# e4s2024/E4S2024

Hardware: AMD Instinct MI355X
Metric: 1024x1024 faces/sec (StyleGAN2 regional synthesis, gen_img) (higher is better)
Workload: dtype f16+mxfp6x2 (masked 3x3 layers >= 32^2) / bf16x3 (all other layers); 1 GPU; BASELINE configs[1]: StyleGAN2 1024x1024 synthesis from random W+, 12-region masks, batch=4/GPU; batch_per_gpu=4, global_batch=4, parallelism=frames x1, streams_per_gpu=2

## Files before the change

### e4s2024_amd/csrc/modconv_uphc.hip

```cpp
#include <stdlib.h>

#include "common.h"
#include "sb_common.h"

using namespace e4s;

namespace {

struct UpHcParams {
    uint4* out;
    const uint4* x;
    const uint4* whi;
    const uint4* wlo;
    const float* d;
    const float* blur;
    const float* noise;
    const float* noise_weight;
    const float* act_bias;
    const float* s_next;
    const float* zeros;
    int noise_bstride, act;
    int bs, cin, cout, h, w;
    int tiles_x, tiles_y;
    int ntile, ncot;
    int exp;
    int rev;
    int walk;
    int64_t plane_in, plane_out;
};

constexpr int HC_T = 16;
constexpr int HC_STEP = HC_T - 2;
constexpr int HC_PW = HC_T + 1, HC_PH = HC_T + 2;
constexpr int HC_PATCH = HC_PW * HC_PH;
constexpr int HC_NT = 512;
constexpr int HC_XB4 = 4 * HC_PATCH;
constexpr int HC_W4 = 36 * 32;
constexpr int HC_BODY = (2 * HC_XB4 + 2 * HC_W4) * 16;
constexpr int HC_EP_D = 0, HC_EP_B = 64, HC_EP_S = 128, HC_EP_FLOATS = 192;
constexpr int HC_LDS = HC_BODY + HC_EP_FLOATS * 4;
constexpr int HC_G = 3;
static_assert(HC_LDS <= 80 * 1024, "two workgroups per CU");

template <int CTRL>
__device__ __forceinline__ float dpp_row(float v) {
    return __builtin_bit_cast(float, __builtin_amdgcn_update_dpp(0, __builtin_bit_cast(int, v), CTRL, 0xf, 0xf, true));
}
constexpr int DPP_ROW_SHL1 = 0x101;
constexpr int DPP_ROW_SHR1 = 0x111;

__device__ __forceinline__ uint4 dpp_row_shr1(uint4 v) {
    uint4 r;
    r.x = (unsigned)__builtin_amdgcn_update_dpp(0, (int)v.x, DPP_ROW_SHR1, 0xf, 0xf, true);
    r.y = (unsigned)__builtin_amdgcn_update_dpp(0, (int)v.y, DPP_ROW_SHR1, 0xf, 0xf, true);
    r.z = (unsigned)__builtin_amdgcn_update_dpp(0, (int)v.z, DPP_ROW_SHR1, 0xf, 0xf, true);
    r.w = (unsigned)__builtin_amdgcn_update_dpp(0, (int)v.w, DPP_ROW_SHR1, 0xf, 0xf, true);
    return r;
}
template <int PAR>
__device__ __forceinline__ void hc_unit(f32x16 (&accs)[4], const uint4* xs, const uint4* whalf) {
    uint4 bh[2], bl[2], ah[2], al[2];
    auto fetch_b = [&](int dyi, int slot) __attribute__((always_inline)) {
        bh[slot] = xs[dyi * HC_PW + 1];
        bl[slot] = xs[2 * HC_PATCH + dyi * HC_PW + 1];
    };
    auto fetch_a = [&](int tap, int slot) __attribute__((always_inline)) {
        ah[slot] = whalf[tap * 64];
        al[slot] = whalf[18 * 32 + tap * 64];
    };
    fetch_b(0, 0);
    fetch_a(0, 0);
#pragma unroll
    for (int dyi = 0; dyi < 3; ++dyi) {
        const int bs = dyi & 1;
        if (dyi + 1 < 3) fetch_b(dyi + 1, bs ^ 1);
        const uint4 sh = dpp_row_shr1(bh[bs]), sl = dpp_row_shr1(bl[bs]);
#pragma unroll
        for (int kx = 0; kx < 3; ++kx) {
            const int tap = dyi * 3 + kx, cs = tap & 1;
            if (tap + 1 < 9) fetch_a(tap + 1, cs ^ 1);
            const uint4 xh = kx == 2 ? sh : bh[bs], xl = kx == 2 ? sl : bl[bs];
            const int ai = 2 * PAR + (kx & 1);
            accs[ai] = __builtin_amdgcn_mfma_f32_32x32x16_bf16(__builtin_bit_cast(bf16x8, ah[cs]), __builtin_bit_cast(bf16x8, xh), accs[ai], 0, 0, 0);
            accs[ai] = __builtin_amdgcn_mfma_f32_32x32x16_bf16(__builtin_bit_cast(bf16x8, ah[cs]), __builtin_bit_cast(bf16x8, xl), accs[ai], 0, 0, 0);
            accs[ai] = __builtin_amdgcn_mfma_f32_32x32x16_bf16(__builtin_bit_cast(bf16x8, al[cs]), __builtin_bit_cast(bf16x8, xh), accs[ai], 0, 0, 0);
            __builtin_amdgcn_sched_barrier(0);
        }
    }
}

E4S_PROF_DECL(g_prof_hc)

__device__ __forceinline__ void hc_epilogue(const UpHcParams& p, const f32x16 (&accs)[4], const unsigned char* lds_raw, int ep_off, const float2 (&nz)[2], bool lane_ok,
                                            int b, int co0, int pm, int pbx, int khalf) {
    const int ho = 2 * p.h, wo = 2 * p.w;
    float khf[4];
    {
        float cs[4], S = 0.f;
#pragma unroll
        for (int cc = 0; cc < 4; ++cc) { cs[cc] = p.blur[cc] + p.blur[4 + cc] + p.blur[8 + cc] + p.blur[12 + cc]; S += cs[cc]; }
        const float rs = 1.f / sqrtf(S);
#pragma unroll
        for (int u = 0; u < 4; ++u) khf[u] = cs[3 - u] * rs;
    }
    const float nw = p.noise ? p.noise_weight[0] : 0.f;
    const float neg = p.act ? 0.2f : 1.f, gain = p.act ? 1.41421356237309515f : 1.f;
    const size_t opl = (size_t)ho * wo;
    const size_t o_base = ((size_t)b * (p.cout >> 3) + (size_t)(co0 >> 3)) * opl + (size_t)(2 * pm) * wo + (size_t)(2 * pbx + khalf);
#pragma unroll
    for (int g = 0; g < 4; ++g) {
        unsigned ep_i = (unsigned)(ep_off / 4 + 8 * g + 4 * khalf);
        asm volatile("" : "+v"(ep_i));
        const float* ep = reinterpret_cast<const float*>(lds_raw) + ep_i;
        const float4 d4 = *reinterpret_cast<const float4*>(ep + HC_EP_D);
        const float4 b4 = *reinterpret_cast<const float4*>(ep + HC_EP_B);
        const float4 s4 = *reinterpret_cast<const float4*>(ep + HC_EP_S);
        const float dd[4] = {d4.x, d4.y, d4.z, d4.w}, bb[4] = {b4.x, b4.y, b4.z, b4.w}, sn[4] = {s4.x, s4.y, s4.z, s4.w};
#pragma unroll
        for (int pa = 0; pa < 2; ++pa) {
            const float nze = __fmul_rn(nw, nz[pa].x), nzo = __fmul_rn(nw, nz[pa].y);
            float ue[4], uo[4];
#pragma unroll
            for (int j = 0; j < 4; ++j) {
                const float z0 = accs[2 * pa][4 * g + j], z1 = accs[2 * pa + 1][4 * g + j];
                const float l1 = dpp_row<DPP_ROW_SHR1>(z1);
                const float r0 = dpp_row<DPP_ROW_SHL1>(z0);
                const float r1 = dpp_row<DPP_ROW_SHL1>(z1);
                float oe = __fmul_rn(khf[0], l1);
                oe = __builtin_fmaf(khf[1], z0, oe);
                oe = __builtin_fmaf(khf[2], z1, oe);
                oe = __builtin_fmaf(khf[3], r0, oe);
                float oo = __fmul_rn(khf[0], z0);
                oo = __builtin_fmaf(khf[1], z1, oo);
                oo = __builtin_fmaf(khf[2], r0, oo);
                oo = __builtin_fmaf(khf[3], r1, oo);
                float ve = __builtin_fmaf(oe, dd[j], bb[j]) + nze, vo = __builtin_fmaf(oo, dd[j], bb[j]) + nzo;
                ve = fmaxf(ve, ve * neg) * gain;
                vo = fmaxf(vo, vo * neg) * gain;
                ue[j] = __fmul_rn(ve, sn[j]);
                uo[j] = __fmul_rn(vo, sn[j]);
            }
            unsigned he[2], le[2], ho_[2], lo_[2];
            split2(ue[0], ue[1], he[0], le[0]);
            split2(ue[2], ue[3], he[1], le[1]);
            split2(uo[0], uo[1], ho_[0], lo_[0]);
            split2(uo[2], uo[3], ho_[1], lo_[1]);
#pragma unroll
            for (int q = 0; q < 2; ++q) {
                auto r = __builtin_amdgcn_permlane32_swap(he[q], ho_[q], false, false);
                he[q] = r[0]; ho_[q] = r[1];
                auto r2 = __builtin_amdgcn_permlane32_swap(le[q], lo_[q], false, false);
                le[q] = r2[0]; lo_[q] = r2[1];
            }
#ifdef E4S_PHASE_PROF
            if ((p.exp & 4) && he[0] != 0x12345678u) continue;
#endif
            if (lane_ok) {
                const size_t o4 = o_base + (size_t)g * opl + (size_t)pa * wo;
                p.out[o4] = make_uint4(he[0], he[1], ho_[0], ho_[1]);
                p.out[(size_t)p.plane_out + o4] = make_uint4(le[0], le[1], lo_[0], lo_[1]);
            }
        }
    }
}


__global__ __launch_bounds__(HC_NT, 4) void up_hc_kernel(const UpHcParams p) {
    extern __shared__ __attribute__((aligned(16))) unsigned char lds_raw[];
    const uint4* lds4 = reinterpret_cast<const uint4*>(lds_raw);
    const float* epw = reinterpret_cast<const float*>(lds_raw + HC_BODY);
    const int tid = threadIdx.x;
    const int lane = tid & 63;
    const int wave = __builtin_amdgcn_readfirstlane(tid >> 6);
    const int l5 = lane & 31, khalf = lane >> 5;
    E4S_PROF_MARK(g_prof_hc, 0);
    const int tyt = blockIdx.x / p.tiles_x, txt = blockIdx.x - tyt * p.tiles_x;
    const int m0 = tyt * HC_T, p0x = txt * HC_STEP - 1;
    const int co0 = blockIdx.y * 32;
    const int b = blockIdx.z;
    const int hw = p.h * p.w, ho = 2 * p.h, wo = 2 * p.w;
    const int nchunk = p.cin >> 4, cb8 = p.cin >> 3;
    const unsigned zero_off = (unsigned)(2 * p.plane_in * 16);

    const int pty = 2 * wave + (l5 >> 4), ptx = l5 & 15;
    const int pm = m0 + pty, pbx = p0x + ptx;
    const bool lane_ok = ptx >= 1 && ptx <= HC_STEP && pbx < p.w && pm < p.h;
    float2 nz[2] = {make_float2(0.f, 0.f), make_float2(0.f, 0.f)};
    if (p.noise && lane_ok) {
        const float* np = p.noise + (size_t)b * p.noise_bstride + (size_t)(2 * pm) * wo + 2 * pbx;
        nz[0] = *reinterpret_cast<const float2*>(np);
        nz[1] = *reinterpret_cast<const float2*>(np + wo);
    }

    unsigned xoffs[3], xdst[3];
    bool xin[3];
#pragma unroll
    for (int k = 0; k < 3; ++k) {
        int u = wave + 8 * k;
        u = u < 20 ? u : 19;
        const int j = u % 5, combo = u / 5;
        const int e = j * 64 + lane;
        const int py = e / HC_PW, px = e - py * HC_PW;
        const int gy = m0 - 1 + py, gx = p0x - 1 + px;
        xin[k] = e < HC_PATCH && gy >= 0 && gy < p.h && gx >= 0 && gx < p.w;
        xoffs[k] = (unsigned)((combo >> 1) * p.plane_in) + (unsigned)((b * cb8 + (combo & 1)) * hw + gy * p.w + gx);
        xdst[k] = (unsigned)((combo * HC_PATCH + j * 64) * 16);
    }
    auto issue_x = [&](int c) __attribute__((always_inline)) {
        const unsigned st = (unsigned)(c & 1) * (unsigned)(HC_XB4 * 16);
#pragma unroll
        for (int k = 0; k < 3; ++k) {
            const int e = ((wave + 8 * k < 20 ? wave + 8 * k : 19) % 5) * 64 + lane;
            if (e < HC_PATCH) dma16_asm(p.x, xin[k] ? (xoffs[k] + (unsigned)(2 * c * hw)) * 16u : zero_off, st + xdst[k]);
        }
    };
    auto issue_w = [&](int u) __attribute__((always_inline)) {
        const unsigned st = (unsigned)((2 * HC_XB4 + (u & 1) * HC_W4) * 16);
        const int c = u >> 1, par = u & 1;
#pragma unroll
        for (int k = 0; k < 3; ++k) {
            int piece = wave + 8 * k;
            piece = piece < 18 ? piece : 17;
            const int hl = piece / 9;
            const int rem = piece * 64 - hl * 576 + lane;
            dma16_asm(hl ? p.wlo : p.whi, (unsigned)(((((par * nchunk + c) * 18 + (rem >> 5)) * p.cout) + co0 + (rem & 31)) * 16), st + (unsigned)(piece * 1024));
        }
    };
    {
        const unsigned co4 = (unsigned)((co0 + l5) * 4);
        dma4_asm(p.d, (unsigned)(b * p.cout * 4) + co4, (unsigned)(HC_BODY + HC_EP_D * 4));
        dma4_asm(p.s_next, (unsigned)(b * p.cout * 4) + co4, (unsigned)(HC_BODY + HC_EP_S * 4));
        dma4_asm(p.act_bias ? p.act_bias : p.zeros, p.act_bias ? co4 : 0u, (unsigned)(HC_BODY + HC_EP_B * 4));
    }
    issue_x(0);
    issue_w(0);
    issue_w(1);
    if (nchunk > 1) issue_x(1);

    const int xoff = pty * HC_PW + ptx;
    f32x16 accs[4];
#pragma unroll
    for (int a = 0; a < 4; ++a)
#pragma unroll
        for (int r = 0; r < 16; ++r) accs[a][r] = 0.f;

#pragma unroll 1
    for (int c = 0; c < nchunk; ++c) {
        const bool last = c + 1 >= nchunk;
#pragma unroll
        for (int par = 0; par < 2; ++par) {
            if (!last) E4S_WAIT_VM(2 * HC_G);
            else if (par == 0) E4S_WAIT_VM(HC_G);
            else E4S_WAIT_VM(0);
            E4S_LDS_BARRIER();
            if (c == 0 && par == 0) E4S_PROF_MARK(g_prof_hc, 1);
            unsigned xb_i = (unsigned)((c & 1) * HC_XB4 + khalf * HC_PATCH + xoff);
            unsigned wb_i = (unsigned)(2 * HC_XB4 + par * HC_W4 + khalf * 32 + l5);
            asm volatile("" : "+v"(xb_i), "+v"(wb_i));
            const uint4* xs = lds4 + xb_i;
            const uint4* whalf = lds4 + wb_i;
            if (par == 0) hc_unit<0>(accs, xs, whalf); else hc_unit<1>(accs, xs, whalf);
            E4S_LDS_BARRIER();
            if (!last) {
                issue_w(2 * c + par + 2);
                if (par == 1 && c + 2 < nchunk) issue_x(c + 2);
            }
        }
    }
    E4S_PROF_MARK(g_prof_hc, 2);

    E4S_PROF_MARK(g_prof_hc, 3);
    if (blockIdx.x == 0 && blockIdx.y == 0 && blockIdx.z == 0 && tid < 1) p.out[(size_t)p.plane_out * 2] = make_uint4(0u, 0u, 0u, 0u);
    hc_epilogue(p, accs, lds_raw, HC_BODY, nz, lane_ok, b, co0, pm, pbx, khalf);
    E4S_PROF_MARK(g_prof_hc, 4);
    E4S_PROF_DRAIN();
    E4S_PROF_MARK(g_prof_hc, 5);
}


constexpr int HP_NCW = 8;
constexpr int HP_NT = 64 * (HP_NCW + 2);
constexpr int HP_NX = 4, HP_NW = 4;
constexpr int HP_W0 = HP_NX * HC_XB4;
constexpr int HP_BODY = (HP_NX * HC_XB4 + HP_NW * HC_W4) * 16;
constexpr int HP_LDS = HP_BODY + HC_EP_FLOATS * 4;
constexpr int HP_GX = 20, HP_GW = 18;
static_assert(HP_LDS <= 160 * 1024 && (HP_NX - 1) * HP_GX <= 63 && (HP_NW - 1) * HP_GW + 3 <= 63, "LDS per CU; vmcnt is a 6-bit counter");

__global__ __launch_bounds__(HP_NT) void up_hcp_kernel(const UpHcParams p) {
    extern __shared__ __attribute__((aligned(16))) unsigned char lds_raw[];
    const uint4* lds4 = reinterpret_cast<const uint4*>(lds_raw);
    const int tid = threadIdx.x;
    const int lane = tid & 63;
    const int wave = __builtin_amdgcn_readfirstlane(tid >> 6);
    const int hw = p.h * p.w, wo = 2 * p.w;
    const int nchunk = p.cin >> 4, NU = 2 * nchunk;
    const int stride = gridDim.x, first = walk_offset(blockIdx.x, stride, p.walk & 1);
    const int my_tiles = (p.ntile - first + stride - 1) / stride;
    const int my_items = my_tiles * p.ncot;
    const int per_img = p.tiles_x * p.tiles_y;
    const int total = my_items * NU;
    auto item_coords = [&](int i, int& b, int& cot, int& tyt, int& txt) __attribute__((always_inline)) {
        i = i < my_items ? i : my_items - 1;
        int t = first + (i / p.ncot) * stride;
        t = p.rev ? p.ntile - 1 - t : t;
        cot = i % p.ncot;
        b = t / per_img;
        walk_tile_xy(t - b * per_img, p.tiles_x, p.tiles_y, p.walk >> 8, tyt, txt);
    };

    if (wave == HP_NCW) {
        lds_byte* const lds_b = (lds_byte*)lds_raw;
        auto issue_w = [&](int k) __attribute__((always_inline)) {
            const int u = k % NU, c = u >> 1, par = u & 1;
            int b, cot, tyt, txt;
            item_coords(k / NU, b, cot, tyt, txt);
            const unsigned wst = (unsigned)((HP_W0 + (k % HP_NW) * HC_W4) * 16);
#pragma unroll
            for (int piece = 0; piece < HP_GW; ++piece) {
                const int hl = piece / 9;
                const int rem = piece * 64 - hl * 576 + lane;
                dma16(hl ? p.wlo : p.whi, (unsigned)(((((par * nchunk + c) * 18 + (rem >> 5)) * p.cout) + cot * 32 + (rem & 31)) * 16), lds_b + wst + piece * 1024);
            }
        };
        auto item_setup = [&](int i) __attribute__((always_inline)) {
            int b, cot, tyt, txt;
            item_coords(i, b, cot, tyt, txt);
            const unsigned co4 = (unsigned)((cot * 32 + (lane & 31)) * 4);
            dma4(p.d, (unsigned)(b * p.cout * 4) + co4, lds_b + HP_BODY + HC_EP_D * 4);
            dma4(p.s_next, (unsigned)(b * p.cout * 4) + co4, lds_b + HP_BODY + HC_EP_S * 4);
            dma4(p.act_bias ? p.act_bias : p.zeros, p.act_bias ? co4 : 0u, lds_b + HP_BODY + HC_EP_B * 4);
        };
        item_setup(0);
#pragma unroll
        for (int k = 0; k < HP_NW - 1; ++k) issue_w(k);
#pragma unroll 1
        for (int k = 0; k < total; ++k) {
            E4S_WAIT_VM(2 * HP_GW);
            E4S_LDS_BARRIER();
            if (k > 0 && k % NU == 0) item_setup(k / NU);
            issue_w(k + HP_NW - 1);
        }
        E4S_WAIT_VM(0);
        return;
    }
    if (wave == HP_NCW + 1) {
        const int cb8 = p.cin >> 3;
        lds_byte* const lds_b = (lds_byte*)lds_raw;
        const unsigned zero_off = (unsigned)(2 * p.plane_in * 16);
        auto issue_x = [&](int q) __attribute__((always_inline)) {
            const int c = q % nchunk;
            int b, cot, tyt, txt;
            item_coords(q / nchunk, b, cot, tyt, txt);
            const unsigned xst = (unsigned)((q % HP_NX) * (HC_XB4 * 16));
            const int m0 = tyt * HC_T, p0x = txt * HC_STEP - 1;
            const unsigned cb0 = (unsigned)((b * cb8 + 2 * c) * hw);
#pragma unroll
            for (int j = 0; j < 5; ++j) {
                const int e = j * 64 + lane;
                const int py = e / HC_PW, px = e - py * HC_PW;
                const int gy = m0 - 1 + py, gx = p0x - 1 + px;
                const bool inb = gy >= 0 && gy < p.h && gx >= 0 && gx < p.w;
                const unsigned pix = (unsigned)(gy * p.w + gx);
                if (e < HC_PATCH) {
#pragma unroll
                    for (int combo = 0; combo < 4; ++combo) {
                        const unsigned cbase = (unsigned)((combo >> 1) * p.plane_in) + cb0 + (unsigned)((combo & 1) * hw);
                        dma16(p.x, inb ? (cbase + pix) * 16u : zero_off, lds_b + xst + (combo * HC_PATCH + j * 64) * 16);
                    }
                }
            }
        };
#pragma unroll
        for (int q = 0; q < HP_NX - 1; ++q) issue_x(q);
#pragma unroll 1
        for (int k = 0; k < total; ++k) {
            if (k & 1) { E4S_LDS_BARRIER(); continue; }
            E4S_WAIT_VM(2 * HP_GX);
            E4S_LDS_BARRIER();
            issue_x((k >> 1) + HP_NX - 1);
        }
        E4S_WAIT_VM(0);
        return;
    }

    const int l5 = lane & 31, khalf = lane >> 5;
    const int pty = 2 * wave + (l5 >> 4), ptx = l5 & 15;
    const int xoff = pty * HC_PW + ptx;
    if (blockIdx.x == 0 && tid < 1) p.out[(size_t)p.plane_out * 2] = make_uint4(0u, 0u, 0u, 0u);
    int xbuf = 0;
#pragma unroll 1
    for (int ti = 0; ti < my_items; ++ti) {
        int b, cot, tyt, txt;
        item_coords(ti, b, cot, tyt, txt);
        const int pm = tyt * HC_T + pty, pbx = txt * HC_STEP - 1 + ptx;
        const bool lane_ok = ptx >= 1 && ptx <= HC_STEP && pbx < p.w && pm < p.h;
        float2 nz[2] = {make_float2(0.f, 0.f), make_float2(0.f, 0.f)};
        if (p.noise && lane_ok) {
            const float* np = p.noise + (size_t)b * p.noise_bstride + (size_t)(2 * pm) * wo + 2 * pbx;
            nz[0] = *reinterpret_cast<const float2*>(np);
            nz[1] = *reinterpret_cast<const float2*>(np + wo);
        }
        f32x16 accs[4];
#pragma unroll
        for (int a = 0; a < 4; ++a)
#pragma unroll
            for (int r = 0; r < 16; ++r) accs[a][r] = 0.f;
#pragma unroll 1
        for (int c = 0; c < nchunk; ++c) {
#pragma unroll
            for (int par = 0; par < 2; ++par) {
                const int k = ti * NU + 2 * c + par;
                E4S_LDS_BARRIER();
                unsigned xb_i = (unsigned)(xbuf * HC_XB4 + khalf * HC_PATCH + xoff);
                unsigned wb_i = (unsigned)(HP_W0 + (k % HP_NW) * HC_W4 + khalf * 32 + l5);
                asm volatile("" : "+v"(xb_i), "+v"(wb_i));
                const uint4* xs = lds4 + xb_i;
                const uint4* whalf = lds4 + wb_i;
#ifdef E4S_PHASE_PROF
                if (p.exp & 2) continue;
#endif
                if (par == 0) hc_unit<0>(accs, xs, whalf); else hc_unit<1>(accs, xs, whalf);
            }
            xbuf = xbuf + 1 < HP_NX ? xbuf + 1 : 0;
        }
#ifdef E4S_PHASE_PROF
        if (p.exp & 1) { asm volatile("" :: "v"(accs[0][0]), "v"(accs[1][0]), "v"(accs[2][0]), "v"(accs[3][0])); continue; }
#endif
        hc_epilogue(p, accs, lds_raw, HP_BODY, nz, lane_ok, b, cot * 32, pm, pbx, khalf);
    }
}

__global__ __launch_bounds__(256) void prep_weights_hc_kernel(uint16_t* __restrict__ whi, uint16_t* __restrict__ wlo, const float* __restrict__ weight,
                                                              const float* __restrict__ blur, int cout, int cin, float scale) {
    const int nchunk = (cin + CKS - 1) / CKS;
    const int64_t total = (int64_t)2 * nchunk * 9 * 2 * cout * 8;
    float kvf[4];
    {
        float rsum[4], S = 0.f;
#pragma unroll
        for (int r = 0; r < 4; ++r) { rsum[r] = blur[4 * r] + blur[4 * r + 1] + blur[4 * r + 2] + blur[4 * r + 3]; S += rsum[r]; }
        const float rs = 1.f / sqrtf(S);
#pragma unroll
        for (int t = 0; t < 4; ++t) kvf[t] = rsum[3 - t] * rs;
    }
    for (int64_t i = (int64_t)blockIdx.x * 256 + threadIdx.x; i < total; i += (int64_t)gridDim.x * 256) {
        const int e = (int)(i & 7);
        int64_t r = i >> 3;
        const int co = (int)(r % cout); r /= cout;
        const int half = (int)(r & 1); r >>= 1;
        const int tap = (int)(r % 9); r /= 9;
        const int chunk = (int)(r % nchunk);
        const int par = (int)(r / nchunk);
        const int ci = chunk * CKS + half * 8 + e;
        float v = 0.f;
        if (ci < cin) {
            const float* w = weight + ((size_t)co * cin + ci) * 9;
            const int dy = tap / 3 - 1, kx = tap % 3;
#pragma unroll
            for (int ky = 0; ky < 3; ++ky) {
                const int ty = ky + 2 * dy + 1 - par;
                if (ty >= 0 && ty <= 3) v += kvf[ty] * w[ky * 3 + kx];
            }
            v *= scale;
        }
        const unsigned hp = pack_bf16_rne(v, 0.f) & 0xffffu;
        const float hf = __builtin_bit_cast(float, hp << 16);
        whi[i] = (uint16_t)hp;
        wlo[i] = (uint16_t)(pack_bf16_rne(v - hf, 0.f) & 0xffffu);
    }
}

__device__ uint4 g_hc_zero[4];

}

#ifdef E4S_PHASE_PROF
extern "C" E4S_API int e4s_prof_read_hc(long long* host, int64_t n) {
    return (int)hipMemcpyFromSymbol(host, HIP_SYMBOL(g_prof_hc), (size_t)n * sizeof(long long), 0, hipMemcpyDeviceToHost);
}
extern "C" E4S_API int e4s_prof_clear_hc() {
    void* ptr = nullptr;
    hipError_t e = hipGetSymbolAddress(&ptr, HIP_SYMBOL(g_prof_hc));
    if (e != hipSuccess) return (int)e;
    return (int)hipMemset(ptr, 0, sizeof(long long) * (size_t)E4S_PROF_BLOCKS * E4S_PROF_SLOTS);
}
#endif

extern "C" int e4s_modconv_prep_weights_hc(uint16_t* whi, uint16_t* wlo, const float* weight, const float* blur, int cout, int cin, void* stream) {
    E4S_REQUIRE(whi && wlo && weight && blur, "modconv_prep_weights_hc: null tensor");
    E4S_REQUIRE(cout >= 1 && cin >= 1, "modconv_prep_weights_hc: bad channel counts");
    const float scale = 1.0f / sqrtf((float)cin * 9.f);
    const int64_t total = (int64_t)2 * cdiv(cin, CKS) * 9 * 2 * cout * 8;
    const int grid = (int)(cdiv64(total, 256) < 4096 ? cdiv64(total, 256) : 4096);
    hipLaunchKernelGGL(prep_weights_hc_kernel, dim3(grid), dim3(256), 0, (hipStream_t)stream, whi, wlo, weight, blur, cout, cin, scale);
    return check_launch("modconv_prep_weights_hc");
}

extern "C" int e4s_modconv_up_hc(uint16_t* out_sp, const uint16_t* x_sp, const uint16_t* whi, const uint16_t* wlo, const float* d, const float* blur,
                                 const float* noise, int noise_bs, const float* noise_weight, const float* act_bias, int act,
                                 int bs, int cin, int cout, int h, int w, const float* s_next, void* stream) {
    E4S_REQUIRE(out_sp && x_sp && whi && wlo && d && blur && s_next, "modconv_up_hc: null tensor (d and s_next are required)");
    E4S_REQUIRE(bs >= 0 && bs <= 65535 && h >= 1 && w >= 1 && cin >= 16 && cin % 16 == 0 && cout >= 32 && cout % 32 == 0, "modconv_up_hc: bad size (cin %% 16, cout %% 32)");
    E4S_REQUIRE((int64_t)bs * cout * 4 * h * w < ((int64_t)1 << 31) && (int64_t)bs * cin * h * w < ((int64_t)1 << 31), "modconv_up_hc: a tensor must stay below 2^31 elements");
    E4S_REQUIRE((((uintptr_t)out_sp | (uintptr_t)x_sp | (uintptr_t)whi | (uintptr_t)wlo) & 15) == 0, "modconv_up_hc: tensors must be 16-byte aligned");
    E4S_REQUIRE(!noise || (noise_weight && (noise_bs == 1 || noise_bs == bs) && ((uintptr_t)noise & 7) == 0), "modconv_up_hc: noise needs its weight, batch 1 or bs and 8-byte alignment");
    if (bs == 0) return 0;
    static const float* zeros = [] {
        void* ptr = nullptr;
        return hipGetSymbolAddress(&ptr, HIP_SYMBOL(g_hc_zero)) == hipSuccess ? static_cast<const float*>(ptr) : nullptr;
    }();
    static const hipError_t attr = hipFuncSetAttribute(reinterpret_cast<const void*>(&up_hc_kernel), hipFuncAttributeMaxDynamicSharedMemorySize, HC_LDS);
    static const hipError_t attr_p = hipFuncSetAttribute(reinterpret_cast<const void*>(&up_hcp_kernel), hipFuncAttributeMaxDynamicSharedMemorySize, HP_LDS);
    if (!zeros || attr != hipSuccess || attr_p != hipSuccess) return fail(E4S_ERR_ARG, "modconv_up_hc: cannot set up the kernel (zero block / dynamic LDS limit)");
    UpHcParams p;
    p.out = reinterpret_cast<uint4*>(out_sp); p.x = reinterpret_cast<const uint4*>(x_sp);
    p.whi = reinterpret_cast<const uint4*>(whi); p.wlo = reinterpret_cast<const uint4*>(wlo);
    p.d = d; p.blur = blur; p.noise = noise; p.noise_weight = noise_weight; p.act_bias = act_bias; p.s_next = s_next; p.zeros = zeros;
    p.noise_bstride = (noise && noise_bs > 1) ? 4 * h * w : 0;
    p.act = act & 1; p.bs = bs; p.cin = cin; p.cout = cout; p.h = h; p.w = w;
    p.tiles_x = cdiv(2 * w, 2 * HC_STEP); p.tiles_y = cdiv(h, HC_T);
    p.ntile = p.tiles_x * p.tiles_y * bs; p.ncot = cout / 32;
    p.plane_in = (int64_t)bs * (cin / 8) * h * w;
    p.plane_out = (int64_t)bs * (cout / 8) * 4 * h * w;
    static const int rev = [] { const char* e = getenv("E4S_HC_REV"); return e ? atoi(e) : 1; }();
    static const int walk = [] { const char* e = getenv("E4S_WALK"); return e ? atoi(e) : (1 | (8 << 8)); }();
    p.rev = rev; p.walk = walk;
#ifdef E4S_PHASE_PROF
    { const char* e = getenv("E4S_HC_EXP"); p.exp = e ? atoi(e) : 0; }
#else
    p.exp = 0;
#endif
    if (cin >= 32) {
        static const int ncu = [] {
            int dev = 0, n = 256;
            if (hipGetDevice(&dev) == hipSuccess) (void)hipDeviceGetAttribute(&n, hipDeviceAttributeMultiprocessorCount, dev);
            return n > 0 ? n : 256;
        }();
        hipLaunchKernelGGL(up_hcp_kernel, dim3(p.ntile < ncu ? p.ntile : ncu), dim3(HP_NT), HP_LDS, (hipStream_t)stream, p);
        return check_launch("modconv_up_hc");
    }
    hipLaunchKernelGGL(up_hc_kernel, dim3(p.tiles_x * p.tiles_y, cout / 32, bs), dim3(HC_NT), HC_LDS, (hipStream_t)stream, p);
    return check_launch("modconv_up_hc");
}
```

Before: 1509 faces/s.

## Use wide 32x8 tiles with wave-level DPP shifts in persistent upsample modconv

The persistent upsample-conv kernel switches from a 16-wide, two-rows-per-wave tile to a 32-wide tile with one tile row per wave. Horizontal neighbour shifts now use wave-wide DPP instead of row DPP, so halo overhead per tile drops and patch loads become whole 64-lane pieces. Leftover tiles are also split at item (tile x cout-tile) granularity across persistent workgroups to balance the tail. Risks include changed LDS footprint, edge handling of wave-wide shifts across the 32-lane halves, and more complex index math.

```diff
diff --git a/e4s2024_amd/csrc/modconv_uphc.hip b/e4s2024_amd/csrc/modconv_uphc.hip
--- a/e4s2024_amd/csrc/modconv_uphc.hip
+++ b/e4s2024_amd/csrc/modconv_uphc.hip
@@ -48,21 +48,37 @@
 }
 constexpr int DPP_ROW_SHL1 = 0x101;
 constexpr int DPP_ROW_SHR1 = 0x111;
-
-__device__ __forceinline__ uint4 dpp_row_shr1(uint4 v) {
+constexpr int DPP_WAVE_SHL1 = 0x130;
+constexpr int DPP_WAVE_SHR1 = 0x138;
+
+constexpr int HP_TW = 32, HP_TH = 8;
+constexpr int HP_STEP = HP_TW - 2;
+constexpr int HP_PW = HP_TW, HP_PH = HP_TH + 2;
+constexpr int HP_PATCH = HP_PW * HP_PH;
+template <bool WIDE> struct HcGeo;
+template <> struct HcGeo<false> {
+    static constexpr int PW = HC_PW, PATCH = HC_PATCH, XO = 1, SHR1 = DPP_ROW_SHR1, SHL1 = DPP_ROW_SHL1;
+};
+template <> struct HcGeo<true> {
+    static constexpr int PW = HP_PW, PATCH = HP_PATCH, XO = 0, SHR1 = DPP_WAVE_SHR1, SHL1 = DPP_WAVE_SHL1;
+};
+
+template <int CTRL>
+__device__ __forceinline__ uint4 dpp_shr1(uint4 v) {
     uint4 r;
-    r.x = (unsigned)__builtin_amdgcn_update_dpp(0, (int)v.x, DPP_ROW_SHR1, 0xf, 0xf, true);
-    r.y = (unsigned)__builtin_amdgcn_update_dpp(0, (int)v.y, DPP_ROW_SHR1, 0xf, 0xf, true);
-    r.z = (unsigned)__builtin_amdgcn_update_dpp(0, (int)v.z, DPP_ROW_SHR1, 0xf, 0xf, true);
-    r.w = (unsigned)__builtin_amdgcn_update_dpp(0, (int)v.w, DPP_ROW_SHR1, 0xf, 0xf, true);
+    r.x = (unsigned)__builtin_amdgcn_update_dpp(0, (int)v.x, CTRL, 0xf, 0xf, true);
+    r.y = (unsigned)__builtin_amdgcn_update_dpp(0, (int)v.y, CTRL, 0xf, 0xf, true);
+    r.z = (unsigned)__builtin_amdgcn_update_dpp(0, (int)v.z, CTRL, 0xf, 0xf, true);
+    r.w = (unsigned)__builtin_amdgcn_update_dpp(0, (int)v.w, CTRL, 0xf, 0xf, true);
     return r;
 }
-template <int PAR>
+template <int PAR, bool WIDE>
 __device__ __forceinline__ void hc_unit(f32x16 (&accs)[4], const uint4* xs, const uint4* whalf) {
+    using G = HcGeo<WIDE>;
     uint4 bh[2], bl[2], ah[2], al[2];
     auto fetch_b = [&](int dyi, int slot) __attribute__((always_inline)) {
-        bh[slot] = xs[dyi * HC_PW + 1];
-        bl[slot] = xs[2 * HC_PATCH + dyi * HC_PW + 1];
+        bh[slot] = xs[dyi * G::PW + G::XO];
+        bl[slot] = xs[2 * G::PATCH + dyi * G::PW + G::XO];
     };
     auto fetch_a = [&](int tap, int slot) __attribute__((always_inline)) {
         ah[slot] = whalf[tap * 64];
@@ -74,7 +90,7 @@
     for (int dyi = 0; dyi < 3; ++dyi) {
         const int bs = dyi & 1;
         if (dyi + 1 < 3) fetch_b(dyi + 1, bs ^ 1);
-        const uint4 sh = dpp_row_shr1(bh[bs]), sl = dpp_row_shr1(bl[bs]);
+        const uint4 sh = dpp_shr1<G::SHR1>(bh[bs]), sl = dpp_shr1<G::SHR1>(bl[bs]);
 #pragma unroll
         for (int kx = 0; kx < 3; ++kx) {
             const int tap = dyi * 3 + kx, cs = tap & 1;
@@ -91,8 +107,10 @@
 
 E4S_PROF_DECL(g_prof_hc)
 
+template <bool WIDE>
 __device__ __forceinline__ void hc_epilogue(const UpHcParams& p, const f32x16 (&accs)[4], const unsigned char* lds_raw, int ep_off, const float2 (&nz)[2], bool lane_ok,
-                                            int b, int co0, int pm, int pbx, int khalf) {
+                                            int b, int co0, int row0, int p0x, int l5, int khalf) {
+    using G = HcGeo<WIDE>;
     const int ho = 2 * p.h, wo = 2 * p.w;
     float khf[4];
     {
@@ -106,7 +124,9 @@
     const float nw = p.noise ? p.noise_weight[0] : 0.f;
     const float neg = p.act ? 0.2f : 1.f, gain = p.act ? 1.41421356237309515f : 1.f;
     const size_t opl = (size_t)ho * wo;
-    const size_t o_base = ((size_t)b * (p.cout >> 3) + (size_t)(co0 >> 3)) * opl + (size_t)(2 * pm) * wo + (size_t)(2 * pbx + khalf);
+    const int64_t o_base = (int64_t)(((size_t)b * (p.cout >> 3) + (size_t)(co0 >> 3)) * opl + (size_t)(2 * row0) * wo) + 2 * p0x;
+    const unsigned o_lane = (unsigned)((WIDE ? 0 : (l5 >> 4) * 2 * wo) + 2 * (WIDE ? l5 : l5 & 15) + khalf) * 16u;
+    unsigned char* const out_b = reinterpret_cast<unsigned char*>(p.out);
 #pragma unroll
     for (int g = 0; g < 4; ++g) {
         unsigned ep_i = (unsigned)(ep_off / 4 + 8 * g + 4 * khalf);
@@ -123,9 +143,9 @@
 #pragma unroll
             for (int j = 0; j < 4; ++j) {
                 const float z0 = accs[2 * pa][4 * g + j], z1 = accs[2 * pa + 1][4 * g + j];
-                const float l1 = dpp_row<DPP_ROW_SHR1>(z1);
-                const float r0 = dpp_row<DPP_ROW_SHL1>(z0);
-                const float r1 = dpp_row<DPP_ROW_SHL1>(z1);
+                const float l1 = dpp_row<G::SHR1>(z1);
+                const float r0 = dpp_row<G::SHL1>(z0);
+                const float r1 = dpp_row<G::SHL1>(z1);
                 float oe = __fmul_rn(khf[0], l1);
                 oe = __builtin_fmaf(khf[1], z0, oe);
                 oe = __builtin_fmaf(khf[2], z1, oe);
@@ -156,9 +176,11 @@
             if ((p.exp & 4) && he[0] != 0x12345678u) continue;
 #endif
             if (lane_ok) {
-                const size_t o4 = o_base + (size_t)g * opl + (size_t)pa * wo;
-                p.out[o4] = make_uint4(he[0], he[1], ho_[0], ho_[1]);
-                p.out[(size_t)p.plane_out + o4] = make_uint4(le[0], le[1], lo_[0], lo_[1]);
+                unsigned char* const ohi = out_b + (o_base + (int64_t)((size_t)g * opl + (size_t)pa * wo)) * 16;
+                unsigned ol = o_lane;
+                asm volatile("" : "+v"(ol));
+                *reinterpret_cast<uint4*>(ohi + ol) = make_uint4(he[0], he[1], ho_[0], ho_[1]);
+                *reinterpret_cast<uint4*>(ohi + p.plane_out * 16 + ol) = make_uint4(le[0], le[1], lo_[0], lo_[1]);
             }
         }
     }
@@ -259,7 +281,7 @@
             asm volatile("" : "+v"(xb_i), "+v"(wb_i));
             const uint4* xs = lds4 + xb_i;
             const uint4* whalf = lds4 + wb_i;
-            if (par == 0) hc_unit<0>(accs, xs, whalf); else hc_unit<1>(accs, xs, whalf);
+            if (par == 0) hc_unit<0, false>(accs, xs, whalf); else hc_unit<1, false>(accs, xs, whalf);
             E4S_LDS_BARRIER();
             if (!last) {
                 issue_w(2 * c + par + 2);
@@ -271,7 +293,7 @@
 
     E4S_PROF_MARK(g_prof_hc, 3);
     if (blockIdx.x == 0 && blockIdx.y == 0 && blockIdx.z == 0 && tid < 1) p.out[(size_t)p.plane_out * 2] = make_uint4(0u, 0u, 0u, 0u);
-    hc_epilogue(p, accs, lds_raw, HC_BODY, nz, lane_ok, b, co0, pm, pbx, khalf);
+    hc_epilogue<false>(p, accs, lds_raw, HC_BODY, nz, lane_ok, b, co0, m0 + 2 * wave, p0x, l5, khalf);
     E4S_PROF_MARK(g_prof_hc, 4);
     E4S_PROF_DRAIN();
     E4S_PROF_MARK(g_prof_hc, 5);
@@ -281,10 +303,13 @@
 constexpr int HP_NCW = 8;
 constexpr int HP_NT = 64 * (HP_NCW + 2);
 constexpr int HP_NX = 4, HP_NW = 4;
-constexpr int HP_W0 = HP_NX * HC_XB4;
-constexpr int HP_BODY = (HP_NX * HC_XB4 + HP_NW * HC_W4) * 16;
+constexpr int HP_XB4 = 4 * HP_PATCH;
+constexpr int HP_W0 = HP_NX * HP_XB4;
+constexpr int HP_BODY = (HP_NX * HP_XB4 + HP_NW * HC_W4) * 16;
 constexpr int HP_LDS = HP_BODY + HC_EP_FLOATS * 4;
-constexpr int HP_GX = 20, HP_GW = 18;
+constexpr int HP_XPIECES = HP_PATCH / 64;
+constexpr int HP_GX = 4 * HP_XPIECES, HP_GW = 18;
+static_assert(HP_NCW == HP_TH && HP_PATCH % 64 == 0, "one compute wave per tile row; whole 64-lane pieces");
 static_assert(HP_LDS <= 160 * 1024 && (HP_NX - 1) * HP_GX <= 63 && (HP_NW - 1) * HP_GW + 3 <= 63, "LDS per CU; vmcnt is a 6-bit counter");
 
 __global__ __launch_bounds__(HP_NT) void up_hcp_kernel(const UpHcParams p) {
@@ -296,15 +321,20 @@
     const int hw = p.h * p.w, wo = 2 * p.w;
     const int nchunk = p.cin >> 4, NU = 2 * nchunk;
     const int stride = gridDim.x, first = walk_offset(blockIdx.x, stride, p.walk & 1);
-    const int my_tiles = (p.ntile - first + stride - 1) / stride;
-    const int my_items = my_tiles * p.ncot;
+    const int full = p.ntile / stride;
+    const int full_items = full * p.ncot;
+    const int rem_items = (p.ntile - full * stride) * p.ncot;
+    const int per = (rem_items + stride - 1) / stride;
+    const int rem_mine = rem_items - first * per;
+    const int my_items = full_items + (rem_mine < 0 ? 0 : rem_mine < per ? rem_mine : per);
     const int per_img = p.tiles_x * p.tiles_y;
     const int total = my_items * NU;
     auto item_coords = [&](int i, int& b, int& cot, int& tyt, int& txt) __attribute__((always_inline)) {
         i = i < my_items ? i : my_items - 1;
-        int t = first + (i / p.ncot) * stride;
+        const int r = i < full_items ? i : first * per + (i - full_items);
+        int t = i < full_items ? first + (r / p.ncot) * stride : full * stride + r / p.ncot;
         t = p.rev ? p.ntile - 1 - t : t;
-        cot = i % p.ncot;
+        cot = r % p.ncot;
         b = t / per_img;
         walk_tile_xy(t - b * per_img, p.tiles_x, p.tiles_y, p.walk >> 8, tyt, txt);
     };
@@ -352,22 +382,20 @@
             const int c = q % nchunk;
             int b, cot, tyt, txt;
             item_coords(q / nchunk, b, cot, tyt, txt);
-            const unsigned xst = (unsigned)((q % HP_NX) * (HC_XB4 * 16));
-            const int m0 = tyt * HC_T, p0x = txt * HC_STEP - 1;
+            const unsigned xst = (unsigned)((q % HP_NX) * (HP_XB4 * 16));
+            const int m0 = tyt * HP_TH, p0x = txt * HP_STEP - 1;
             const unsigned cb0 = (unsigned)((b * cb8 + 2 * c) * hw);
 #pragma unroll
-            for (int j = 0; j < 5; ++j) {
+            for (int j = 0; j < HP_XPIECES; ++j) {
                 const int e = j * 64 + lane;
-                const int py = e / HC_PW, px = e - py * HC_PW;
-                const int gy = m0 - 1 + py, gx = p0x - 1 + px;
+                const int py = e / HP_PW, px = e - py * HP_PW;
+                const int gy = m0 - 1 + py, gx = p0x + px;
                 const bool inb = gy >= 0 && gy < p.h && gx >= 0 && gx < p.w;
                 const unsigned pix = (unsigned)(gy * p.w + gx);
-                if (e < HC_PATCH) {
-#pragma unroll
-                    for (int combo = 0; combo < 4; ++combo) {
-                        const unsigned cbase = (unsigned)((combo >> 1) * p.plane_in) + cb0 + (unsigned)((combo & 1) * hw);
-                        dma16(p.x, inb ? (cbase + pix) * 16u : zero_off, lds_b + xst + (combo * HC_PATCH + j * 64) * 16);
-                    }
+#pragma unroll
+                for (int combo = 0; combo < 4; ++combo) {
+                    const unsigned cbase = (unsigned)((combo >> 1) * p.plane_in) + cb0 + (unsigned)((combo & 1) * hw);
+                    dma16(p.x, inb ? (cbase + pix) * 16u : zero_off, lds_b + xst + (combo * HP_PATCH + j * 64) * 16);
                 }
             }
         };
@@ -385,16 +413,16 @@
     }
 
     const int l5 = lane & 31, khalf = lane >> 5;
-    const int pty = 2 * wave + (l5 >> 4), ptx = l5 & 15;
-    const int xoff = pty * HC_PW + ptx;
+    const int pty = wave, ptx = l5;
+    const int xoff = pty * HP_PW + ptx;
     if (blockIdx.x == 0 && tid < 1) p.out[(size_t)p.plane_out * 2] = make_uint4(0u, 0u, 0u, 0u);
     int xbuf = 0;
 #pragma unroll 1
     for (int ti = 0; ti < my_items; ++ti) {
         int b, cot, tyt, txt;
         item_coords(ti, b, cot, tyt, txt);
-        const int pm = tyt * HC_T + pty, pbx = txt * HC_STEP - 1 + ptx;
-        const bool lane_ok = ptx >= 1 && ptx <= HC_STEP && pbx < p.w && pm < p.h;
+        const int pm = tyt * HP_TH + pty, p0x = txt * HP_STEP - 1, pbx = p0x + ptx;
+        const bool lane_ok = ptx >= 1 && ptx <= HP_STEP && pbx < p.w && pm < p.h;
         float2 nz[2] = {make_float2(0.f, 0.f), make_float2(0.f, 0.f)};
         if (p.noise && lane_ok) {
             const float* np = p.noise + (size_t)b * p.noise_bstride + (size_t)(2 * pm) * wo + 2 * pbx;
@@ -412,7 +440,7 @@
             for (int par = 0; par < 2; ++par) {
                 const int k = ti * NU + 2 * c + par;
                 E4S_LDS_BARRIER();
-                unsigned xb_i = (unsigned)(xbuf * HC_XB4 + khalf * HC_PATCH + xoff);
+                unsigned xb_i = (unsigned)(xbuf * HP_XB4 + khalf * HP_PATCH + xoff);
                 unsigned wb_i = (unsigned)(HP_W0 + (k % HP_NW) * HC_W4 + khalf * 32 + l5);
                 asm volatile("" : "+v"(xb_i), "+v"(wb_i));
                 const uint4* xs = lds4 + xb_i;
@@ -420,14 +448,14 @@
 #ifdef E4S_PHASE_PROF
                 if (p.exp & 2) continue;
 #endif
-                if (par == 0) hc_unit<0>(accs, xs, whalf); else hc_unit<1>(accs, xs, whalf);
+                if (par == 0) hc_unit<0, true>(accs, xs, whalf); else hc_unit<1, true>(accs, xs, whalf);
             }
             xbuf = xbuf + 1 < HP_NX ? xbuf + 1 : 0;
         }
 #ifdef E4S_PHASE_PROF
         if (p.exp & 1) { asm volatile("" :: "v"(accs[0][0]), "v"(accs[1][0]), "v"(accs[2][0]), "v"(accs[3][0])); continue; }
 #endif
-        hc_epilogue(p, accs, lds_raw, HP_BODY, nz, lane_ok, b, cot * 32, pm, pbx, khalf);
+        hc_epilogue<true>(p, accs, lds_raw, HP_BODY, nz, lane_ok, b, cot * 32, pm, p0x, l5, khalf);
     }
 }
 
@@ -519,7 +547,8 @@
     p.d = d; p.blur = blur; p.noise = noise; p.noise_weight = noise_weight; p.act_bias = act_bias; p.s_next = s_next; p.zeros = zeros;
     p.noise_bstride = (noise && noise_bs > 1) ? 4 * h * w : 0;
     p.act = act & 1; p.bs = bs; p.cin = cin; p.cout = cout; p.h = h; p.w = w;
-    p.tiles_x = cdiv(2 * w, 2 * HC_STEP); p.tiles_y = cdiv(h, HC_T);
+    const bool persistent = cin >= 32;
+    p.tiles_x = cdiv(w, persistent ? HP_STEP : HC_STEP); p.tiles_y = cdiv(h, persistent ? HP_TH : HC_T);
     p.ntile = p.tiles_x * p.tiles_y * bs; p.ncot = cout / 32;
     p.plane_in = (int64_t)bs * (cin / 8) * h * w;
     p.plane_out = (int64_t)bs * (cout / 8) * 4 * h * w;
@@ -531,7 +560,7 @@
 #else
     p.exp = 0;
 #endif
-    if (cin >= 32) {
+    if (persistent) {
         static const int ncu = [] {
             int dev = 0, n = 256;
             if (hipGetDevice(&dev) == hipSuccess) (void)hipDeviceGetAttribute(&n, hipDeviceAttributeMultiprocessorCount, dev);
```

New measurement: 1528 faces/s (median of 6 runs). 1.2% higher.
